# davidfang00/opticalflowdiffusion

Hardware: AMD Instinct MI355X
Metric: UNet denoise steps/sec @ 2x436x1024 flow, bs=16 (higher is better)
Workload: dtype bf16

## Files before the change

opticalflowdiffusion_amd/csrc/conv_pc.hip:

```cpp
#include <cstdlib>
#include <type_traits>
#include "conv_common.h"

namespace ofd {

namespace wp {

struct PcCfg {
    using C = Cfg<2, 2>;
    static constexpr int NPROD = C::NTHREADS, XPT = C::XPT;
    static constexpr int WSLOT = FRAGS * 2 * 1024;
    static constexpr int MAX_ITEMS = 512;
    static constexpr int ITEMS_OFF = 2 * C::XB + 2 * WSLOT;
    static constexpr int LDS_BYTES = ITEMS_OFF + MAX_ITEMS * 16;
};

template <bool PRO>
__global__ void __launch_bounds__(512, 2) conv3x3_pc_kernel(const ConvParams P) {
    using C = PcCfg::C;
    constexpr int NPROD = PcCfg::NPROD, XPT = PcCfg::XPT;
    extern __shared__ __attribute__((aligned(16))) unsigned char smem[];
    unsigned char* const wlds = smem + 2 * C::XB;
    const int tid = threadIdx.x;

    const int tiles_y = (P.H + C::ROWS - 1) / C::ROWS;
    const int tpi = P.tiles_x * tiles_y, ntiles = tpi * P.B, ny = P.Cout / C::BN, G = gridDim.x;
    const int nitems = (ntiles + 7) / 8 * 8 * ny;
    const int n32 = P.total_chunks * 2;
    auto decode = [&](int j, int& b, int& oy0, int& ox0, int& cy) -> bool {
        if (j >= nitems) return false;
        const int g = j >> 3;
        cy = ny > 1 ? g % ny : 0;
        int tile = (ny > 1 ? g / ny : g) * 8 + (j & 7);
        if (tile >= ntiles) return false;
        tile = xcd_tile_order(tile, ntiles);
        b = tile / tpi;
        const int t_in = tile - b * tpi;
        oy0 = (t_in / P.tiles_x) * C::ROWS;
        ox0 = (t_in % P.tiles_x) * TW;
        return true;
    };
    const int nit = blockIdx.x < nitems ? min((nitems - 1 - (int)blockIdx.x) / G + 1, PcCfg::MAX_ITEMS) : 0;
    int4* const items = (int4*)(smem + PcCfg::ITEMS_OFF);
    for (int k = tid; k < nit; k += 512) {
        int b_, y_, x_, c_;
        const bool ok = decode(blockIdx.x + k * G, b_, y_, x_, c_);
        items[k] = make_int4(ok ? b_ : -1, y_, x_, c_);
    }
    __syncthreads();
    int nvalid_items = 0;
    if (nit > 0) {
        int lo = 0, hi = nit;
        while (lo < hi) { const int mid = (lo + hi) >> 1; if (items[mid].x >= 0) lo = mid + 1; else hi = mid; }
        nvalid_items = lo;
    }
    const int T = n32 * nvalid_items;
    if (T == 0) return;
    auto item_at = [&](int k, int& b, int& oy0, int& ox0, int& cy) -> bool {
        if (k >= nvalid_items) return false;
        const int4 d = items[k];
        b = __builtin_amdgcn_readfirstlane(d.x); oy0 = __builtin_amdgcn_readfirstlane(d.y);
        ox0 = __builtin_amdgcn_readfirstlane(d.z); cy = __builtin_amdgcn_readfirstlane(d.w);
        return true;
    };

    if (tid >= 256) {
        const int ptid = tid - 256;
        const int c8 = ptid % NC;
        int tyx[XPT];
#pragma unroll
        for (int i = 0; i < XPT; ++i) {
            const int p = min(ptid / NC + i * (NPROD / NC), C::NPIX - 1);
            const int ty = p / IW;
            tyx[i] = (ty << 8) | (p - ty * IW);
        }
        int lk = 0, lkc = 0, lb, loy0, lox0, lcy;
        item_at(0, lb, loy0, lox0, lcy);
        auto advance = [&]() {
            if (++lkc == n32) {
                if (item_at(lk + 1, lb, loy0, lox0, lcy)) { lkc = 0; ++lk; }
                else lkc = n32 - 1;
            }
        };
        auto issue = [&](u4 (&xs)[XPT], unsigned& okmask, float (&ps)[8], float (&pb)[8]) {
            const int k64 = lkc >> 1;
            int si = 0, first = 0;
            while (k64 >= first + P.src[si].chunks) { first += P.src[si].chunks; ++si; }
            const ConvSrcDev& S = P.src[si];
            const bf16_t* base = S.ptr + (size_t)lb * S.SH * S.SW * S.src_channels + S.ch_offset + (k64 - first) * 64 + (lkc & 1) * CK + c8 * 8;
            const int up = S.mode == 1 ? 1 : 0;
            okmask = 0;
#pragma unroll
            for (int i = 0; i < XPT; ++i) {
                const int iy = loy0 - 1 + (tyx[i] >> 8), ix = lox0 - 1 + (tyx[i] & 0xff);
                const bool ok = iy >= 0 && iy < P.H && ix >= 0 && ix < P.W;
                okmask |= (ok ? 1u : 0u) << i;
                const int sy = min(max(iy, 0), P.H - 1) >> up, sx = min(max(ix, 0), P.W - 1) >> up;
                xs[i] = *(const u4*)(base + ((size_t)sy * S.SW + sx) * S.src_channels);
            }
            if constexpr (PRO) load_in_affine8(P, lb, lkc * CK, c8 * 8, ps, pb);
        };
        auto stage = [&](const u4 (&xs)[XPT], const unsigned okmask, const float (&ps)[8], const float (&pb)[8], unsigned char* xbuf) {
            stage_write<C, PRO>(xs, okmask, ps, pb, xbuf, ptid);
        };
        const int pw = __builtin_amdgcn_readfirstlane(ptid >> 6), plane_ = ptid & 63;
        const int cin8 = P.Cin_total / 8;
        const unsigned wlds_addr = (unsigned)(size_t)(__attribute__((address_space(3))) unsigned char*)wlds;
        int held0 = -1, held1 = -1;
        int sk = 0, skc = 0, scy, sb_, sy_, sx_;
        item_at(0, sb_, sy_, sx_, scy);
        auto stage_advance = [&]() {
            if (++skc == n32) {
                if (item_at(sk + 1, sb_, sy_, sx_, scy)) { skc = 0; ++sk; }
                else skc = n32 - 1;
            }
        };
        auto weights_dma = [&](const int slot) -> bool {
            const int key = (scy << 16) | skc;
            int& held = slot ? held1 : held0;
            if (held == key) return false;
            held = key;
#pragma unroll
            for (int q = 0; q < FRAGS * 2 / 4; ++q) {
                const int fr = pw * (FRAGS * 2 / 4) + q, fi = fr >> 1, ns_ = fr & 1;
                const int g = fi / 3, ky = fi - g * 3, ks = g / 3, kx = g - ks * 3;
                const int row = (ky * 3 + kx) * cin8 + skc * NC + ks * 2;
                const bf16_t* sbase = P.weight + ((size_t)row * P.Cout + scy * C::BN + 32 * ns_) * 8;
                const unsigned dst = wlds_addr + (unsigned)(((slot * FRAGS + fi) * 2 + ns_) * 1024);
                const unsigned voff = (unsigned)(((plane_ >> 5) * P.Cout + (plane_ & 31)) * 16);
                asm volatile("s_mov_b32 m0, %0\n\ts_nop 0\n\tglobal_load_lds_dwordx4 %1, %2" :: "s"(dst), "v"(voff), "s"(sbase) : "memory");
            }
            return true;
        };
        u4 x0[XPT], x1[XPT], x2[XPT];
        unsigned ok0 = 0, ok1 = 0, ok2 = 0;
        float ps0[8], pb0[8], ps1[8], pb1[8], ps2[8], pb2[8];
        weights_dma(0); stage_advance();
        issue(x0, ok0, ps0, pb0); advance();
        issue(x1, ok1, ps1, pb1); advance();
        issue(x2, ok2, ps2, pb2); advance();
        stage(x0, ok0, ps0, pb0, smem);
        asm volatile("s_waitcnt vmcnt(0)" ::: "memory");
        __syncthreads();
#define PC_STEP(XL, OKL, PSL, PBL, XS, OKS, PSS, PBS, BUF)                                          \
        {                                                                                           \
            if (i >= T) break;                                                                      \
            const bool wd_ = weights_dma(BUF);                  \
            stage_advance();                                                                        \
            issue(XL, OKL, PSL, PBL);                                                               \
            stage(XS, OKS, PSS, PBS, smem + (BUF) * C::XB);                                         \
            advance();                                                                              \
            if (wd_) asm volatile("s_waitcnt vmcnt(%0)" ::"n"(XPT + (PRO ? 4 : 0)) : "memory");     \
            __syncthreads();                                                                        \
            ++i;                                                                                    \
        }
        for (int i = 0; i < T;) {
            PC_STEP(x0, ok0, ps0, pb0, x1, ok1, ps1, pb1, 1)
            PC_STEP(x1, ok1, ps1, pb1, x2, ok2, ps2, pb2, 0)
            PC_STEP(x2, ok2, ps2, pb2, x0, ok0, ps0, pb0, 1)
            PC_STEP(x0, ok0, ps0, pb0, x1, ok1, ps1, pb1, 0)
            PC_STEP(x1, ok1, ps1, pb1, x2, ok2, ps2, pb2, 1)
            PC_STEP(x2, ok2, ps2, pb2, x0, ok0, ps0, pb0, 0)
        }
#undef PC_STEP
        return;
    }

    const int lane = tid & 63, wave = __builtin_amdgcn_readfirstlane(tid >> 6);
    const int l31 = lane & 31, half = lane >> 5;
    const int ns = wave & 1, ph = wave >> 1;
    __builtin_amdgcn_s_setprio(2);

    int ik = 0, b, oy0, ox0, cy;
    item_at(0, b, oy0, ox0, cy);

    f32x16 biasv;
    auto load_bias = [&](int cy_) {
#pragma unroll
        for (int g = 0; g < 4; ++g) {
            const float4 b4 = P.bias ? *(const float4*)(P.bias + cy_ * C::BN + 32 * ns + 8 * g + 4 * half) : make_float4(0.f, 0.f, 0.f, 0.f);
            biasv[4 * g] = b4.x; biasv[4 * g + 1] = b4.y; biasv[4 * g + 2] = b4.z; biasv[4 * g + 3] = b4.w;
        }
    };
    load_bias(cy);
    f32x16 acc[8];

    const int xrow_off = half * C::US + (8 * ph * IW + l31) * 16;
    const unsigned char* const wfrag = wlds + ns * 1024 + lane * 16;
    auto chunk = [&](const int slot, const unsigned char* xbase, auto first_tag) {
        constexpr bool FIRST = decltype(first_tag)::value;
        const unsigned char* xrow = xbase + xrow_off;
#pragma unroll
        for (int g = 0; g < 6; ++g) {
            const int ks = g / 3, kx = g % 3;
            bf16x8 x[10];
#pragma unroll
            for (int jr = 0; jr < 10; ++jr) x[jr] = *(const bf16x8*)(xrow + (jr * IW + kx) * 16 + ks * 2 * C::US);
            bf16x8 a[3];
#pragma unroll
            for (int ky = 0; ky < 3; ++ky) a[ky] = *(const bf16x8*)(wfrag + (slot * FRAGS + g * 3 + ky) * 2048);
#pragma unroll
            for (int r = 0; r < 8; ++r)
#pragma unroll
                for (int ky = 0; ky < 3; ++ky)
                    acc[r] = __builtin_amdgcn_mfma_f32_32x32x16_bf16(a[ky], x[r + ky], (FIRST && g == 0 && ky == 0) ? biasv : acc[r], 0, 0, 0);
        }
    };

    const int tiles8 = (P.H + 7) / 8;
    __syncthreads();
    while (true) {
        int nb, noy0, nox0, ncy;
        const bool nvalid = item_at(ik + 1, nb, noy0, nox0, ncy);
        for (int kc = 0; kc < n32; kc += 2) {
            if (kc == 0) chunk(0, smem, std::true_type{}); else chunk(0, smem, std::false_type{});
            __syncthreads();
            chunk(1, smem + C::XB, std::false_type{});
            __syncthreads();
        }
        __builtin_amdgcn_s_setprio(0);
        float stat[8];
#pragma unroll
        for (int i = 0; i < 8; ++i) stat[i] = 0.0f;
        const int oyb = oy0 + 8 * ph, ox = ox0 + l31, cb = cy * C::BN + 32 * ns;
        const bool okx = ox < P.W;
        const size_t oplane_b = (size_t)P.H * P.W * P.Cout * 2;
        const __amdgpu_buffer_rsrc_t orsrc = __builtin_amdgcn_make_buffer_rsrc((void*)(P.out + (size_t)b * P.H * P.W * P.Cout), 0, (int)oplane_b, 0x00020000);
        const unsigned olane = (unsigned)(((min(oyb, P.H - 1) * P.W + min(ox, P.W - 1)) * P.Cout + cb + 8 * half) * 2);
        const unsigned ostride_b = (unsigned)(P.W * P.Cout * 2);
        const bool full = ox0 + TW <= P.W && oyb + 8 <= P.H && oplane_b < (1ull << 31);
        if (full) {
#pragma unroll
            for (int r = 0; r < 8; ++r) {
                uint2 q[4];
#pragma unroll
                for (int g = 0; g < 4; ++g) {
                    q[g] = make_uint2(f2bf2(acc[r][4 * g], acc[r][4 * g + 1]), f2bf2(acc[r][4 * g + 2], acc[r][4 * g + 3]));
                    if (P.gn_partial) gn_stat_add(q[g], stat[g * 2], stat[g * 2 + 1]);
                }
#pragma unroll
                for (int g = 0; g < 4; g += 2) {
                    const auto rx = __builtin_amdgcn_permlane32_swap(q[g].x, q[g + 1].x, false, false);
                    const auto ry = __builtin_amdgcn_permlane32_swap(q[g].y, q[g + 1].y, false, false);
                    u4 pk = {rx[0], ry[0], rx[1], ry[1]};
                    __builtin_amdgcn_raw_buffer_store_b128(pk, orsrc, (int)olane, (int)(r * ostride_b + 16 * g), 0);
                }
            }
        } else {
        bf16_t* orow = P.out + (((size_t)b * P.H + min(oyb, P.H - 1)) * P.W + min(ox, P.W - 1)) * P.Cout + cb + 8 * half;
        const size_t ostride = (size_t)P.W * P.Cout;
#pragma unroll
        for (int r = 0; r < 8; ++r) {
            const bool ok = okx && oyb + r < P.H;
            uint2 q[4];
#pragma unroll
            for (int g = 0; g < 4; ++g) {
                q[g] = make_uint2(f2bf2(acc[r][4 * g], acc[r][4 * g + 1]), f2bf2(acc[r][4 * g + 2], acc[r][4 * g + 3]));
                if (P.gn_partial && ok) gn_stat_add(q[g], stat[g * 2], stat[g * 2 + 1]);
            }
#pragma unroll
            for (int g = 0; g < 4; g += 2) {
                const auto rx = __builtin_amdgcn_permlane32_swap(q[g].x, q[g + 1].x, false, false);
                const auto ry = __builtin_amdgcn_permlane32_swap(q[g].y, q[g + 1].y, false, false);
                if (ok) *(uint4*)(orow + 8 * g) = make_uint4(rx[0], ry[0], rx[1], ry[1]);
            }
            orow += ostride;
        }
        }
        if (P.gn_partial) gn_partial_store_wave<2, C::BN / 8>(P, stat, b, oy0 / 8 + ph, tiles8, ox0 / TW, ns, cy * C::BN / 8, lane);
        if (!nvalid) break;
        ++ik; b = nb; oy0 = noy0; ox0 = nox0;
        if (ncy != cy) { cy = ncy; load_bias(cy); }
        __builtin_amdgcn_s_setprio(2);
    }
}

static bool pc_serves(const ConvParams& P) {
    for (int i = 0; i < P.n_src; ++i)
        if (P.src[i].mode != 0 && P.src[i].mode != 1) return false;
    return P.Cout % 64 == 0 && plain_epilogue(P) && P.W <= 8160 ;
}

}

int launch_conv3x3_pc(const ConvParams& P, hipStream_t s) {
    using namespace wp;
    using C = PcCfg::C;
    if (!pc_serves(P)) return 1;
    static int cus = 0;
    if (!cus) {
        int dev = 0, n = 0;
        OFD_HIP(hipGetDevice(&dev));
        OFD_HIP(hipDeviceGetAttribute(&n, hipDeviceAttributeMultiprocessorCount, dev));
        OFD_HIP(hipFuncSetAttribute((const void*)conv3x3_pc_kernel<false>, hipFuncAttributeMaxDynamicSharedMemorySize, PcCfg::LDS_BYTES));
        OFD_HIP(hipFuncSetAttribute((const void*)conv3x3_pc_kernel<true>, hipFuncAttributeMaxDynamicSharedMemorySize, PcCfg::LDS_BYTES));
        cus = n / 8 * 8 < 8 ? 8 : n / 8 * 8;
    }
    const int tiles_y = (P.H + C::ROWS - 1) / C::ROWS;
    const int ntiles = P.tiles_x * tiles_y * P.B, ny = P.Cout / C::BN;
    const int nitems = (ntiles + 7) / 8 * 8 * ny;
    const int grid = nitems < cus ? nitems : cus;
    if ((long)grid * PcCfg::MAX_ITEMS < nitems) return 1;
    if (P.in_scale) conv3x3_pc_kernel<true><<<grid, 512, PcCfg::LDS_BYTES, s>>>(P);
    else conv3x3_pc_kernel<false><<<grid, 512, PcCfg::LDS_BYTES, s>>>(P);
    OFD_LAUNCH_CHECK();
    return OFD_OK;
}

}
```

Measured before the change: 35.32.

## Switch producer-consumer conv to 16x16x32 MFMA with register-prefetched LDS reads

Replaces the 32x32x16 bf16 MFMA path in the warp-specialized 3x3 conv with 16x16x32 MFMAs, splitting accumulators into 8x2x2 f32x4 tiles. It changes the weight fragment layout in the DMA producer to match. It also software-pipelines LDS reads: the next group's input and weight fragments are loaded into registers while the current MFMAs run, with sched barriers and a single sync per chunk. The epilogue, bias init and GroupNorm partial reduction are rewritten for the new lane layout. This adds register pressure and riskier scheduling under the 2-block launch bound.

After: 35.64, median of 6. Within noise of the previous version (+0.9%).

```diff
diff --git a/opticalflowdiffusion_amd/csrc/conv_pc.hip b/opticalflowdiffusion_amd/csrc/conv_pc.hip
--- a/opticalflowdiffusion_amd/csrc/conv_pc.hip
+++ b/opticalflowdiffusion_amd/csrc/conv_pc.hip
@@ -14,6 +14,32 @@
     static constexpr int ITEMS_OFF = 2 * C::XB + 2 * WSLOT;
     static constexpr int LDS_BYTES = ITEMS_OFF + MAX_ITEMS * 16;
 };
+
+typedef __attribute__((ext_vector_type(4))) float f32x4;
+
+__device__ __forceinline__ void gn_partial_store_pc16(const ConvParams& P, float (&st)[2][2], int b, int ty8, int tiles8, int tx, int ns, int oct0, int lane) {
+#pragma unroll
+    for (int h = 0; h < 2; ++h)
+#pragma unroll
+        for (int k = 0; k < 2; ++k) {
+            float v = st[h][k];
+            v += __uint_as_float(__builtin_amdgcn_mov_dpp(__float_as_uint(v), 0xb1 , 0xf, 0xf, false));
+            v += __uint_as_float(__builtin_amdgcn_mov_dpp(__float_as_uint(v), 0x4e , 0xf, 0xf, false));
+            v += __uint_as_float(__builtin_amdgcn_mov_dpp(__float_as_uint(v), 0x141 , 0xf, 0xf, false));
+            v += __uint_as_float(__builtin_amdgcn_mov_dpp(__float_as_uint(v), 0x140 , 0xf, 0xf, false));
+            const auto r = __builtin_amdgcn_permlane16_swap(__float_as_uint(v), __float_as_uint(v), false, false);
+            st[h][k] = __uint_as_float(r[0]) + __uint_as_float(r[1]);
+        }
+    if (ty8 < tiles8) {
+        const int m = lane >> 5, i = lane & 31, which = i & 1, h = (i >> 1) & 1, slot_i = (i >> 2) & 1, o = (i >> 3 & 1) * 4 + h * 2 + m;
+        const float t00 = st[0][0], t01 = st[0][1], t10 = st[1][0], t11 = st[1][1];
+        const float total = h ? (which ? t11 : t10) : (which ? t01 : t00);
+        if (i < 16) {
+            const bool own = slot_i == 0 && (o >> 2) == ns;
+            P.gn_partial[gn_partial_index(b, tiles8 * P.tiles_x * 4, (ty8 * P.tiles_x + tx) * 4 + ns + slot_i * 2, P.Cout / 8, oct0 + o) + which] = own ? total : 0.0f;
+        }
+    }
+}
 
 template <bool PRO>
 __global__ void __launch_bounds__(512, 2) conv3x3_pc_kernel(const ConvParams P) {
@@ -123,11 +149,11 @@
 #pragma unroll
             for (int q = 0; q < FRAGS * 2 / 4; ++q) {
                 const int fr = pw * (FRAGS * 2 / 4) + q, fi = fr >> 1, ns_ = fr & 1;
-                const int g = fi / 3, ky = fi - g * 3, ks = g / 3, kx = g - ks * 3;
-                const int row = (ky * 3 + kx) * cin8 + skc * NC + ks * 2;
-                const bf16_t* sbase = P.weight + ((size_t)row * P.Cout + scy * C::BN + 32 * ns_) * 8;
+                const int t = fi >> 1, h = fi & 1, kx = t / 3, ky = t - kx * 3;
+                const int row = (ky * 3 + kx) * cin8 + skc * NC;
+                const bf16_t* sbase = P.weight + ((size_t)row * P.Cout + scy * C::BN + 32 * ns_ + 16 * h) * 8;
                 const unsigned dst = wlds_addr + (unsigned)(((slot * FRAGS + fi) * 2 + ns_) * 1024);
-                const unsigned voff = (unsigned)(((plane_ >> 5) * P.Cout + (plane_ & 31)) * 16);
+                const unsigned voff = (unsigned)(((plane_ >> 4) * P.Cout + (plane_ & 15)) * 16);
                 asm volatile("s_mov_b32 m0, %0\n\ts_nop 0\n\tglobal_load_lds_dwordx4 %1, %2" :: "s"(dst), "v"(voff), "s"(sbase) : "memory");
             }
             return true;
@@ -167,107 +193,136 @@
     }
 
     const int lane = tid & 63, wave = __builtin_amdgcn_readfirstlane(tid >> 6);
-    const int l31 = lane & 31, half = lane >> 5;
     const int ns = wave & 1, ph = wave >> 1;
     __builtin_amdgcn_s_setprio(2);
 
     int ik = 0, b, oy0, ox0, cy;
     item_at(0, b, oy0, ox0, cy);
-
-    f32x16 biasv;
+    const int tiles8 = (P.H + 7) / 8;
+
+    const int l15 = lane & 15, lg = lane >> 4;
+    f32x4 bias4[2];
     auto load_bias = [&](int cy_) {
 #pragma unroll
-        for (int g = 0; g < 4; ++g) {
-            const float4 b4 = P.bias ? *(const float4*)(P.bias + cy_ * C::BN + 32 * ns + 8 * g + 4 * half) : make_float4(0.f, 0.f, 0.f, 0.f);
-            biasv[4 * g] = b4.x; biasv[4 * g + 1] = b4.y; biasv[4 * g + 2] = b4.z; biasv[4 * g + 3] = b4.w;
+        for (int h = 0; h < 2; ++h) {
+            const float4 b4 = P.bias ? *(const float4*)(P.bias + cy_ * C::BN + 32 * ns + 16 * h + 4 * lg) : make_float4(0.f, 0.f, 0.f, 0.f);
+            bias4[h][0] = b4.x; bias4[h][1] = b4.y; bias4[h][2] = b4.z; bias4[h][3] = b4.w;
         }
     };
     load_bias(cy);
-    f32x16 acc[8];
-
-    const int xrow_off = half * C::US + (8 * ph * IW + l31) * 16;
+    f32x4 acc[8][2][2];
+
+    const int xrow_off = lg * C::US + (8 * ph * IW + l15) * 16;
     const unsigned char* const wfrag = wlds + ns * 1024 + lane * 16;
-    auto chunk = [&](const int slot, const unsigned char* xbase, auto first_tag) {
-        constexpr bool FIRST = decltype(first_tag)::value;
-        const unsigned char* xrow = xbase + xrow_off;
-#pragma unroll
-        for (int g = 0; g < 6; ++g) {
-            const int ks = g / 3, kx = g % 3;
-            bf16x8 x[10];
-#pragma unroll
-            for (int jr = 0; jr < 10; ++jr) x[jr] = *(const bf16x8*)(xrow + (jr * IW + kx) * 16 + ks * 2 * C::US);
-            bf16x8 a[3];
-#pragma unroll
-            for (int ky = 0; ky < 3; ++ky) a[ky] = *(const bf16x8*)(wfrag + (slot * FRAGS + g * 3 + ky) * 2048);
-#pragma unroll
-            for (int r = 0; r < 8; ++r)
-#pragma unroll
-                for (int ky = 0; ky < 3; ++ky)
-                    acc[r] = __builtin_amdgcn_mfma_f32_32x32x16_bf16(a[ky], x[r + ky], (FIRST && g == 0 && ky == 0) ? biasv : acc[r], 0, 0, 0);
-        }
-    };
-
-    const int tiles8 = (P.H + 7) / 8;
+    bf16x8 xa[6], xb[6], w[6];
+    auto read_x = [&](bf16x8 (&x)[6], const unsigned char* xrow, const int g) {
+        const int kx = g >> 2, p = (g >> 1) & 1, hf = g & 1;
+#pragma unroll
+        for (int j = 0; j < 6; ++j) x[j] = *(const bf16x8*)(xrow + ((4 * hf + j) * IW + kx + 16 * p) * 16);
+    };
+    auto read_w = [&](const int i, const unsigned char* wslot, const int kx) {
+        w[i] = *(const bf16x8*)(wslot + (kx * 6 + i) * 2048);
+    };
+    auto chunk = [&](const int c) {
+        constexpr int FENCE = 0x72;
+        const unsigned char* xrow = smem + xrow_off + (c & 1) * C::XB;
+        const unsigned char* xnext = smem + xrow_off + (~c & 1) * C::XB;
+        const unsigned char* wcur = wfrag + (c & 1) * PcCfg::WSLOT;
+        const unsigned char* wnext = wfrag + (~c & 1) * PcCfg::WSLOT;
+        auto group = [&](const int g, const bf16x8 (&cur)[6], bf16x8 (&nxt)[6]) {
+            const int kx = g >> 2, p = (g >> 1) & 1, hf = g & 1;
+            const bool refill = (g & 3) == 3;
+            __builtin_amdgcn_sched_barrier(FENCE);
+            if (g == 11) __syncthreads();
+            if (g == 11) __builtin_amdgcn_sched_barrier(FENCE);
+            if (g < 11) read_x(nxt, xrow, g + 1); else read_x(nxt, xnext, 0);
+            __builtin_amdgcn_sched_barrier(FENCE);
+#pragma unroll
+            for (int ky = 0; ky < 3; ++ky) {
+#pragma unroll
+                for (int h = 0; h < 2; ++h)
+#pragma unroll
+                    for (int r = 0; r < 4; ++r)
+                        acc[4 * hf + r][p][h] = __builtin_amdgcn_mfma_f32_16x16x32_bf16(w[ky * 2 + h], cur[r + ky], acc[4 * hf + r][p][h], 0, 0, 0);
+                if (refill) {
+                    __builtin_amdgcn_sched_barrier(FENCE);
+                    read_w(ky * 2, g == 11 ? wnext : wcur, g == 11 ? 0 : kx + 1);
+                    read_w(ky * 2 + 1, g == 11 ? wnext : wcur, g == 11 ? 0 : kx + 1);
+                    __builtin_amdgcn_sched_barrier(FENCE);
+                }
+            }
+        };
+#pragma unroll
+        for (int g = 0; g < 12; g += 2) {
+            group(g, xa, xb);
+            group(g + 1, xb, xa);
+        }
+    };
+    auto read_first = [&]() {
+        read_x(xa, smem + xrow_off, 0);
+#pragma unroll
+        for (int i = 0; i < 6; ++i) read_w(i, wfrag, 0);
+    };
+
     __syncthreads();
+    read_first();
     while (true) {
         int nb, noy0, nox0, ncy;
         const bool nvalid = item_at(ik + 1, nb, noy0, nox0, ncy);
-        for (int kc = 0; kc < n32; kc += 2) {
-            if (kc == 0) chunk(0, smem, std::true_type{}); else chunk(0, smem, std::false_type{});
-            __syncthreads();
-            chunk(1, smem + C::XB, std::false_type{});
-            __syncthreads();
-        }
+#pragma unroll
+        for (int r = 0; r < 8; ++r)
+#pragma unroll
+            for (int q = 0; q < 4; ++q) acc[r][q >> 1][q & 1] = bias4[q & 1];
+#pragma nounroll
+        for (int c = 0; c < n32; ++c) chunk(c);
         __builtin_amdgcn_s_setprio(0);
-        float stat[8];
-#pragma unroll
-        for (int i = 0; i < 8; ++i) stat[i] = 0.0f;
-        const int oyb = oy0 + 8 * ph, ox = ox0 + l31, cb = cy * C::BN + 32 * ns;
-        const bool okx = ox < P.W;
+        float st[2][2] = {{0.0f, 0.0f}, {0.0f, 0.0f}};
+        int lane_e = lane;
+        asm volatile("" : "+v"(lane_e));
+        const int l15e = lane_e & 15, lge = lane_e >> 4;
+        const int oyb = oy0 + 8 * ph, ox = ox0 + l15e, cs = cy * C::BN + 32 * ns + 16 * (lge & 1) + 8 * (lge >> 1);
         const size_t oplane_b = (size_t)P.H * P.W * P.Cout * 2;
         const __amdgpu_buffer_rsrc_t orsrc = __builtin_amdgcn_make_buffer_rsrc((void*)(P.out + (size_t)b * P.H * P.W * P.Cout), 0, (int)oplane_b, 0x00020000);
-        const unsigned olane = (unsigned)(((min(oyb, P.H - 1) * P.W + min(ox, P.W - 1)) * P.Cout + cb + 8 * half) * 2);
-        const unsigned ostride_b = (unsigned)(P.W * P.Cout * 2);
+        const unsigned olane = (unsigned)(((min(oyb, P.H - 1) * P.W + min(ox, P.W - 1)) * P.Cout + cs) * 2);
+        const unsigned ostride_b = (unsigned)(P.W * P.Cout * 2), ohalf_b = (unsigned)(16 * P.Cout * 2);
         const bool full = ox0 + TW <= P.W && oyb + 8 <= P.H && oplane_b < (1ull << 31);
+        auto pack = [&](const int r, const int p, const bool ok) -> u4 {
+            uint2 q[2];
+#pragma unroll
+            for (int h = 0; h < 2; ++h) {
+                const f32x4 a = acc[r][p][h];
+                q[h] = make_uint2(f2bf2(a[0], a[1]), f2bf2(a[2], a[3]));
+                if (ok) gn_stat_add(q[h], st[h][0], st[h][1]);
+            }
+            const auto rx = __builtin_amdgcn_permlane16_swap(q[0].x, q[1].x, false, false);
+            const auto ry = __builtin_amdgcn_permlane16_swap(q[0].y, q[1].y, false, false);
+            return u4{rx[0], ry[0], rx[1], ry[1]};
+        };
         if (full) {
 #pragma unroll
             for (int r = 0; r < 8; ++r) {
-                uint2 q[4];
-#pragma unroll
-                for (int g = 0; g < 4; ++g) {
-                    q[g] = make_uint2(f2bf2(acc[r][4 * g], acc[r][4 * g + 1]), f2bf2(acc[r][4 * g + 2], acc[r][4 * g + 3]));
-                    if (P.gn_partial) gn_stat_add(q[g], stat[g * 2], stat[g * 2 + 1]);
+#pragma unroll
+                for (int p = 0; p < 2; ++p)
+                    __builtin_amdgcn_raw_buffer_store_b128(pack(r, p, true), orsrc, (int)olane, (int)(r * ostride_b + p * ohalf_b), 0);
+                __builtin_amdgcn_sched_barrier(0);
+            }
+        } else {
+#pragma unroll
+            for (int r = 0; r < 8; ++r) {
+#pragma unroll
+                for (int p = 0; p < 2; ++p) {
+                    const bool ok = oyb + r < P.H && ox + 16 * p < P.W;
+                    const u4 pk = pack(r, p, ok);
+                    bf16_t* o = P.out + (((size_t)b * P.H + min(oyb + r, P.H - 1)) * P.W + min(ox + 16 * p, P.W - 1)) * P.Cout + cs;
+                    if (ok) *(u4*)o = pk;
                 }
-#pragma unroll
-                for (int g = 0; g < 4; g += 2) {
-                    const auto rx = __builtin_amdgcn_permlane32_swap(q[g].x, q[g + 1].x, false, false);
-                    const auto ry = __builtin_amdgcn_permlane32_swap(q[g].y, q[g + 1].y, false, false);
-                    u4 pk = {rx[0], ry[0], rx[1], ry[1]};
-                    __builtin_amdgcn_raw_buffer_store_b128(pk, orsrc, (int)olane, (int)(r * ostride_b + 16 * g), 0);
-                }
-            }
-        } else {
-        bf16_t* orow = P.out + (((size_t)b * P.H + min(oyb, P.H - 1)) * P.W + min(ox, P.W - 1)) * P.Cout + cb + 8 * half;
-        const size_t ostride = (size_t)P.W * P.Cout;
-#pragma unroll
-        for (int r = 0; r < 8; ++r) {
-            const bool ok = okx && oyb + r < P.H;
-            uint2 q[4];
-#pragma unroll
-            for (int g = 0; g < 4; ++g) {
-                q[g] = make_uint2(f2bf2(acc[r][4 * g], acc[r][4 * g + 1]), f2bf2(acc[r][4 * g + 2], acc[r][4 * g + 3]));
-                if (P.gn_partial && ok) gn_stat_add(q[g], stat[g * 2], stat[g * 2 + 1]);
-            }
-#pragma unroll
-            for (int g = 0; g < 4; g += 2) {
-                const auto rx = __builtin_amdgcn_permlane32_swap(q[g].x, q[g + 1].x, false, false);
-                const auto ry = __builtin_amdgcn_permlane32_swap(q[g].y, q[g + 1].y, false, false);
-                if (ok) *(uint4*)(orow + 8 * g) = make_uint4(rx[0], ry[0], rx[1], ry[1]);
-            }
-            orow += ostride;
-        }
-        }
-        if (P.gn_partial) gn_partial_store_wave<2, C::BN / 8>(P, stat, b, oy0 / 8 + ph, tiles8, ox0 / TW, ns, cy * C::BN / 8, lane);
+                __builtin_amdgcn_sched_barrier(0);
+            }
+        }
+        __builtin_amdgcn_sched_barrier(0);
+        read_first();
+        __builtin_amdgcn_sched_barrier(0);
+        if (P.gn_partial) gn_partial_store_pc16(P, st, b, oy0 / 8 + ph, tiles8, ox0 / TW, ns, cy * C::BN / 8, lane_e);
         if (!nvalid) break;
         ++ik; b = nb; oy0 = noy0; ox0 = nox0;
         if (ncy != cy) { cy = ncy; load_bias(cy); }
```
